# dataexplorations2026/cough_detector

Hardware: AMD Instinct MI355X
Metric: 1s@16kHz clips/sec (featurise+infer) (higher is better)
Workload: dtype bf16x3: split-bf16 MFMA (feature image, activations and BN-folded weights as hi+lo bf16 pairs, 3 v_mfma_f32_32x32x16_bf16 per k-step, f32 accumulate, f32 activations in HBM); featuriser f32

## Files before the change

### cough_detector_amd/csrc/resblock_x3.h

```cpp
#pragma once
#include <utility>

#include "common.h"
#include "nn_common.h"
#include "resnet_plan.h"

namespace cough {
namespace {

#ifdef COUGH_K1_STAMPS
__device__ unsigned long long* g_rb_stamp_buf = nullptr;
#define RB_STAMP(slot)                                                                        \
    do {                                                                                      \
        if (g_rb_stamp_buf && threadIdx.x == 0)                                               \
            g_rb_stamp_buf[(size_t)blockIdx.x * 8 + (slot)] = __builtin_amdgcn_s_memtime();   \
    } while (0)
#else
#define RB_STAMP(slot) do { } while (0)
#endif

struct RbxArgs {
    const float* x;
    int n_clips;
    const bf16_t* wf;
    const float* b1;
    const float* b2;
    float* out;
    const float* fcw;
    const float* fcb;
    float* logits;
    float* probs;
    int* preds;
    const int* nanflag;
};

template <int CIN, int COUT, int G, int XH, int XW>
struct RbxCfg {
    static constexpr int WAVES = 4, THREADS = 256;
    static constexpr bool T16 = rbx_t16(CIN, COUT, XH);
    static constexpr int OH = (XH - 1) / 2 + 1, OW = (XW - 1) / 2 + 1;
    static constexpr int NPX = XH * XW, PER = OH * OW, M = G * PER;
    static constexpr int NT = COUT / 32, MG = WAVES / NT, TILES = (M + 31) / 32;
    static constexpr int MW = (TILES + MG - 1) / MG;
    static constexpr int KS1 = 9 * CIN / 16, KSP = CIN / 16, KS2 = 9 * COUT / 16, KS = KS1 + KSP + KS2;
    static constexpr int CT = COUT / 16 / WAVES, NP = (M + 15) / 16;
    static constexpr int KQ1 = 9 * CIN / 32, KQP = CIN / 32, KQ2 = 9 * COUT / 32, KQ = KQ1 + KQP + KQ2;
    static_assert(!T16 || ((CT == 1 || CT == 2) && COUT == 16 * CT * WAVES && (CIN == 32 || CIN == 64) && G <= 2 &&
                           PER >= 16),
                  "T16: one or two 16-channel tiles per wave, one or two k32-steps per conv1 tap, at most one 16-pixel "
                  "tile straddling two clips");
    static constexpr int CHI = CIN / 8, CHO = COUT / 8;
    static constexpr int RE = (XH + 1) / 2, RO = XH / 2;
    static constexpr int NPP = 2 * XH * OW;
    static constexpr int PB01 = RE * OW, PB10 = 2 * RE * OW, PB11 = 2 * RE * OW + RO * OW;
    static constexpr int NPPC = T16 && G > 1 ? PER + (NPP - PER + 15) / 16 * 16 : NPP;
    static constexpr int ZC = T16 ? 16 : 1;
    static constexpr int CPX = !T16 ? (G * NPP + 1) * 16 : CHI == 4 ? (G * NPPC * 16 + 255) / 256 * 256 : (G * NPPC * 16 + 63) / 64 * 64;
    static constexpr int xoff(int c) {
        if (!T16 || CHI == 4) return c * CPX;
        const int s = (c & 1) * 4 + (c >> 1);
        return 256 + s * CPX + (s >= 2 ? 256 : 0) + (s >= 6 ? 256 : 0);
    }
    static constexpr int ZX = !T16 ? G * NPP * 16 : CHI == 4 ? 4 * CPX : 0;
    static constexpr int KX = T16 && CHI == 8 ? xoff(4) - xoff(0) : 0;
    static constexpr int ZH = T16 ? (M * 16 + 255) / 256 * 256 : M * 16;
    static constexpr int CPH = ZH + ZC * 16;
    static constexpr int XBYTES = !T16 ? CHI * CPX : CHI == 4 ? 4 * CPX + 256 : xoff(7) + CPX, HBYTES = CHO * CPH;
    static_assert(!T16 || (ZX % 256 == 0 && CPH % 256 == 0 && (G == 1 || (NPPC - PER) % 16 == 0)), "T16 bank residues");
    static_assert(!T16 || CHI == 4 || ((xoff(1) - xoff(0)) % 256 == 0 && (xoff(3) - xoff(2)) % 256 == 0 &&
                                       xoff(5) - xoff(1) == KX && xoff(6) - xoff(2) == KX && xoff(7) - xoff(3) == KX &&
                                       xoff(0) >= ZX + 256 && xoff(2) + CPX <= ZX + KX && xoff(4) >= ZX + KX + 256),
                  "T16 x layout, CIN = 64");
    static constexpr int PL = (((XBYTES > HBYTES ? XBYTES : HBYTES) + 255) / 256) * 256;
    static constexpr int BIAS = 2 * PL;
    static constexpr int HRED = BIAS + 2 * COUT * 4;
    static constexpr int LDS = HRED + WAVES * 2 * 4;
    static constexpr int OP = COUT + 4;
    static_assert(T16 || (WAVES % NT == 0 && MG * MW * 32 >= M), "tile split");
    static_assert(OW == (XW + 1) / 2, "sub-image row pitch");
    static_assert(M * OP * 4 <= 2 * PL, "the output tile lies over the planes");
    static constexpr int STAGE_MAX = 18;
    static_assert((G * NPX * CIN / 4 + THREADS - 1) / THREADS <= 2 * STAGE_MAX, "staging registers (f32 input, two batches)");
    static_assert(LDS <= 160 * 1024, "one workgroup must fit a CU");
    static_assert(LDS <= 80 * 1024 || (CIN == 32 && XH > 24) || (CIN == 64 && XH == 12), "two workgroups per CU");
};

template <int CIN, int COUT, int G, int XH, int XW>
__global__ __launch_bounds__(256, 2) void resblock_x3_kernel(RbxArgs a) {
    using Cfg = RbxCfg<CIN, COUT, G, XH, XW>;
    constexpr int THREADS = Cfg::THREADS, OH = Cfg::OH, OW = Cfg::OW, NPX = Cfg::NPX, PER = Cfg::PER, M = Cfg::M;
    constexpr bool T16 = Cfg::T16;
    using f32x4 = __attribute__((ext_vector_type(4))) float;
    constexpr int CHI = Cfg::CHI, CHO = Cfg::CHO, PL = Cfg::PL, OP = Cfg::OP, CPX = Cfg::CPX, CPH = Cfg::CPH, NPP = Cfg::NPP;
    constexpr int ZX = Cfg::ZX, KX = Cfg::KX, ZH = Cfg::ZH, ZC = Cfg::ZC, NPPC = Cfg::NPPC;
#ifndef RBX_D
#define RBX_D 4
#endif
#ifndef RBX_DQ
#define RBX_DQ 3
#endif
#ifndef RBX_P
#define RBX_P 2
#endif
#ifndef RBX_PRIO
#define RBX_PRIO 0
#endif
    extern __shared__ __attribute__((aligned(256))) char smem[];
    float* lbias = reinterpret_cast<float*>(smem + Cfg::BIAS);

    const int tid = threadIdx.x, lane = tid & 63, wave = tid >> 6;
    const int clip0 = blockIdx.x * G;
    const int nvalid = a.n_clips - clip0 < G ? a.n_clips - clip0 : G;
    RB_STAMP(0);

    float bv1 = 0.f, bv2 = 0.f;
    if (tid < COUT) { bv1 = a.b1[tid]; bv2 = a.b2[tid]; }

    constexpr int CT = T16 ? Cfg::CT : 1;
    constexpr int DW = !T16 ? RBX_D : CT == 2 && G == 1 ? 2 : RBX_DQ;
    const bf16_t* wbase = a.wf + size_t(T16 ? wave * CT : wave % Cfg::NT) * 1024 + lane * 8;
    constexpr int WSTEP = T16 ? COUT / 16 : Cfg::NT;
    auto wfrag = [&](int s, int ct, int plane) -> bf16x8 {
        return *reinterpret_cast<const bf16x8*>(wbase + ((size_t(s) * WSTEP + ct) * 2 + plane) * 512);
    };
    bf16x8 ring[DW][CT][2];
#pragma unroll
    for (int i = 0; i < DW; ++i)
#pragma unroll
        for (int ct = 0; ct < CT; ++ct) { ring[i][ct][0] = wfrag(i, ct, 0); ring[i][ct][1] = wfrag(i, ct, 1); }

    {
        constexpr int NPIECE = G * NPX * CIN / 4, UN = (NPIECE + THREADS - 1) / THREADS, QP = CIN / 4;
        constexpr int NB = UN <= Cfg::STAGE_MAX ? 1 : 2, UNB = (UN + NB - 1) / NB;
        const int valid = nvalid * NPX * QP;
        const float4* src = reinterpret_cast<const float4*>(a.x + (long long)clip0 * NPX * CIN);
        if constexpr (T16) {
            constexpr int NZ = CHI / 4;
            if (tid < 2 * NZ * ZC) {
                const int k = tid / ZC;
                *reinterpret_cast<uint4*>(smem + (k / NZ) * PL + ZX + (k % NZ) * KX + (tid % ZC) * 16) = make_uint4(0, 0, 0, 0);
            }
        } else if (tid < 2 * CHI) {
            *reinterpret_cast<uint4*>(smem + (tid / CHI) * PL + (tid % CHI) * CPX + ZX) = make_uint4(0, 0, 0, 0);
        }
#pragma unroll
        for (int b0 = 0; b0 < UN; b0 += UNB) {
            float4 v[UNB];
#pragma unroll
            for (int u = 0; u < UNB; ++u) {
                const int i = tid + (b0 + u) * THREADS;
                v[u] = src[i < valid ? i : valid - 1];
            }
#pragma unroll
            for (int u = 0; u < UNB; ++u) {
                const int i = tid + (b0 + u) * THREADS;
                if (i < NPIECE) {
                    const int P = i / QP, q = i % QP;
                    const int g = P / NPX, rem = P % NPX, ih = rem / XW, iw = rem % XW;
                    const int cell = g * NPPC + ((ih & 1) ? ((iw & 1) ? Cfg::PB11 : Cfg::PB10) : ((iw & 1) ? Cfg::PB01 : 0)) +
                                     (ih >> 1) * OW + (iw >> 1);
                    uint2 hi, lo;
                    if (i >= valid) v[u] = make_float4(0.f, 0.f, 0.f, 0.f);
                    split4(v[u].x, v[u].y, v[u].z, v[u].w, hi, lo);
                    const int off = Cfg::xoff(q >> 1) + cell * 16 + (q & 1) * 8;
                    *reinterpret_cast<uint2*>(smem + off) = hi;
                    *reinterpret_cast<uint2*>(smem + off + PL) = lo;
                }
            }
        }
    }
    if (tid < COUT) { lbias[tid] = bv1; lbias[COUT + tid] = bv2; }
    float fw0 = 0.f, fw1 = 0.f, fb0 = 0.f, fb1 = 0.f;
    if constexpr (COUT == 128) {
        if (a.fcw != nullptr) {
            fw0 = a.fcw[tid & 127]; fw1 = a.fcw[128 + (tid & 127)];
            fb0 = a.fcb[0]; fb1 = a.fcb[1];
        }
    }
    int nan_clip = 0;
    if constexpr (COUT == 128) {
        if (a.fcw != nullptr && a.nanflag != nullptr && (tid & 127) == 0 && (tid >> 7) < nvalid) nan_clip = a.nanflag[clip0 + (tid >> 7)];
    }

    auto tapx = [](int kh, int kw) constexpr -> int {
        const int a = (kh + 1) & 1, b = (kw + 1) & 1;
        return (a ? (b ? Cfg::PB11 : Cfg::PB10) : (b ? Cfg::PB01 : 0)) - (kh == 0 ? Cfg::OW : 0) - (kw == 0 ? 1 : 0);
    };

    constexpr int NT = Cfg::NT, MW = Cfg::MW, KS1 = Cfg::KS1, KSP = Cfg::KSP, KS = Cfg::KS, D = DW;
    const int r = lane & 31, h = lane >> 5, ng = wave % NT, mg = wave / NT;
    int goh[MW], gow[MW], px1[MW], ph1[MW];
    bool rok[MW];
#pragma unroll
    for (int mt = 0; mt < MW; ++mt) {
        const int R = (mg * MW + mt) * 32 + r;
        rok[mt] = R < M;
        const int Rc = rok[mt] ? R : 0;
        const int g = Rc / PER, rem = Rc % PER;
        goh[mt] = rok[mt] ? rem / OW : -4;
        gow[mt] = rem % OW;
        px1[mt] = (g * NPP + rem) * 16 + h * CPX;
        ph1[mt] = Rc * 16 + h * CPH;
    }

    constexpr int NP = Cfg::NP, KQ1 = Cfg::KQ1, KQP = Cfg::KQP, KQ = Cfg::KQ, P = RBX_P, NB = P + 1;
    constexpr int NI = KQ * NP, I2 = (KQ1 + KQP) * NP;
    const int px = lane & 15, tq = lane >> 4, n0 = 16 * CT * wave + 4 * tq;
    unsigned vm[NP];
#pragma unroll
    for (int t = 0; t < NP; ++t) {
        const int R = 16 * t + px, rem = G > 1 ? R % PER : R, oh = rem / OW, ow = rem % OW;
        unsigned m = 0;
#pragma unroll
        for (int tap = 0; tap < 9; ++tap) {
            const int kh = tap / 3, kw = tap % 3;
            const int ih = 2 * oh - 1 + kh, iw = 2 * ow - 1 + kw, jh = oh - 1 + kh, jw = ow - 1 + kw;
            if (unsigned(ih) < unsigned(XH) && unsigned(iw) < unsigned(XW)) m |= 1u << tap;
            if (unsigned(jh) < unsigned(OH) && unsigned(jw) < unsigned(OW)) m |= 1u << (9 + tap);
        }
        vm[t] = R < M ? m : 0u;
    }
    constexpr int DX = (NPPC - PER) * 16;
    const int lbx = px * 16 + Cfg::xoff(tq), lbh = px * 16 + tq * CPH, zh = ZH + tq * CPH;
    const int lbs = lbx + (G > 1 && px >= PER % 16 ? DX : 0);
    const int rx = px + (CHI == 4 ? 0 : Cfg::xoff(tq) / 16);
    auto zcell = [&](int z, int res) { return z + (res & 15) * 16; };
    RB_STAMP(1);
    __syncthreads();
    RB_STAMP(2);
#if RBX_PRIO
    __builtin_amdgcn_s_setprio(1);
#endif

    auto body16 = [&]() {
        f32x4 acc1[CT][NP], acc2[CT][NP];
#pragma unroll
        for (int ct = 0; ct < CT; ++ct)
#pragma unroll
            for (int t = 0; t < NP; ++t) { acc1[ct][t] = f32x4{0.f, 0.f, 0.f, 0.f}; acc2[ct][t] = f32x4{0.f, 0.f, 0.f, 0.f}; }

        int tadr[NP];
        auto aaddr = [&](auto ic) -> const char* {
            constexpr int i = decltype(ic)::value, q = i / NP, t = i % NP;
            constexpr bool conv1 = q < KQ1, proj = !conv1 && q < KQ1 + KQP;
            constexpr int kt = (conv1 ? q : proj ? q - KQ1 : q - KQ1 - KQP) * 32;
            constexpr int C = (conv1 || proj) ? CIN : COUT;
            constexpr int tap = proj ? 4 : kt / C, c32 = (kt % C) / 32, kh = tap / 3, kw = tap % 3;
            if constexpr (c32 == 0) {
                if constexpr (conv1 || proj) {
                    constexpr bool strad = G > 1 && 16 * t < PER && 16 * t + 16 > PER;
                    constexpr int off = 256 * t + (G > 1 && 16 * t >= PER ? DX : 0) + 16 * tapx(kh, kw);
                    tadr[t] = (vm[t] & (1u << tap)) ? (strad ? lbs : lbx) + off : zcell(ZX, rx + tapx(kh, kw));
                } else {
                    constexpr int off = 256 * t + 16 * ((kh - 1) * OW + kw - 1);
                    tadr[t] = (vm[t] & (1u << (9 + tap))) ? lbh + off : zcell(zh, px + (kh - 1) * OW + kw - 1);
                }
            }
            return smem + tadr[t] + c32 * ((conv1 || proj) ? KX : 4 * CPH);
        };
        bf16x8 af[NB][2];
        auto fetch = [&](auto ic) {
            constexpr int i = decltype(ic)::value;
            const char* p = aaddr(ic);
            af[i % NB][0] = *reinterpret_cast<const bf16x8*>(p);
            af[i % NB][1] = *reinterpret_cast<const bf16x8*>(p + PL);
        };
        [&]<int... Js>(std::integer_sequence<int, Js...>) {
            (fetch(std::integral_constant<int, Js>{}), ...);
        }(std::make_integer_sequence<int, P>{});

        auto pair = [&]<int i>() {
            constexpr int q = i / NP, t = i % NP, j = i + P;
            if constexpr (i == I2) {
                RB_STAMP(3);
#if RBX_PRIO
                __builtin_amdgcn_s_setprio(0);
#endif
                __syncthreads();
                for (int z = tid; z < 2 * CHO * ZC; z += THREADS) {
                    const int pl = z / ZC;
                    *reinterpret_cast<uint4*>(smem + (pl / CHO) * PL + (pl % CHO) * CPH + ZH + (z % ZC) * 16) =
                        make_uint4(0, 0, 0, 0);
                }
#pragma unroll
                for (int ct = 0; ct < CT; ++ct) {
                    const int n = n0 + 16 * ct;
                    const float4 bb = *reinterpret_cast<const float4*>(lbias + n);
#pragma unroll
                    for (int u = 0; u < NP; ++u) {
                        const int R = 16 * u + px;
                        uint2 hi, lo;
                        split4(fmaxf(acc1[ct][u][0] + bb.x, 0.f), fmaxf(acc1[ct][u][1] + bb.y, 0.f),
                               fmaxf(acc1[ct][u][2] + bb.z, 0.f), fmaxf(acc1[ct][u][3] + bb.w, 0.f), hi, lo);
                        if (R < M) {
                            const int off = (n >> 3) * CPH + R * 16 + ((n >> 2) & 1) * 8;
                            *reinterpret_cast<uint2*>(smem + off) = hi;
                            *reinterpret_cast<uint2*>(smem + off + PL) = lo;
                        }
                    }
                }
                __syncthreads();
                RB_STAMP(4);
#if RBX_PRIO
                __builtin_amdgcn_s_setprio(1);
#endif
                [&]<int... Js>(std::integer_sequence<int, Js...>) {
                    (fetch(std::integral_constant<int, I2 + Js>{}), ...);
                }(std::make_integer_sequence<int, P>{});
            }
            constexpr bool pf = j < NI && (j < I2) == (i < I2);
            constexpr bool wl = t == NP - 1 && q + DW < KQ;
            const bf16x8 cur_hi = af[i % NB][0], cur_lo = af[i % NB][1];
            const char* np = nullptr;
            if constexpr (pf) np = aaddr(std::integral_constant<int, j>{});
            [&]<int... Ms>(std::integer_sequence<int, Ms...>) {
                ([&] {
                    constexpr int m = Ms, kind = m / CT, ct = m % CT;
                    const bf16x8 w = ring[q % DW][ct][kind == 2 ? 1 : 0];
                    const bf16x8 x = kind == 1 ? cur_lo : cur_hi;
                    __builtin_amdgcn_sched_barrier(0);
                    if constexpr (q < KQ1) acc1[ct][t] = __builtin_amdgcn_mfma_f32_16x16x32_bf16(w, x, acc1[ct][t], 0, 0, 0);
                    else acc2[ct][t] = __builtin_amdgcn_mfma_f32_16x16x32_bf16(w, x, acc2[ct][t], 0, 0, 0);
                    __builtin_amdgcn_sched_barrier(0);
                    if constexpr (pf && m == CT - 1) af[j % NB][0] = *reinterpret_cast<const bf16x8*>(np);
                    if constexpr (pf && m == 2 * CT - 1) af[j % NB][1] = *reinterpret_cast<const bf16x8*>(np + PL);
                    if constexpr (wl && kind == 1) ring[q % DW][ct][0] = wfrag(q + DW, ct, 0);
                    if constexpr (wl && kind == 2) ring[q % DW][ct][1] = wfrag(q + DW, ct, 1);
                }(), ...);
            }(std::make_integer_sequence<int, 3 * CT>{});
            __builtin_amdgcn_sched_barrier(0);
        };
        [&]<int... Is>(std::integer_sequence<int, Is...>) {
            (pair.template operator()<Is>(), ...);
        }(std::make_integer_sequence<int, NI>{});

        RB_STAMP(5);
#if RBX_PRIO
        __builtin_amdgcn_s_setprio(0);
#endif
        __syncthreads();
        float* otile = reinterpret_cast<float*>(smem);
#pragma unroll
        for (int ct = 0; ct < CT; ++ct) {
            const int n = n0 + 16 * ct;
            const float4 bb = *reinterpret_cast<const float4*>(lbias + COUT + n);
#pragma unroll
            for (int t = 0; t < NP; ++t) {
                const int R = 16 * t + px;
                const float4 o = make_float4(fmaxf(acc2[ct][t][0] + bb.x, 0.f), fmaxf(acc2[ct][t][1] + bb.y, 0.f),
                                             fmaxf(acc2[ct][t][2] + bb.z, 0.f), fmaxf(acc2[ct][t][3] + bb.w, 0.f));
                if (R < M) *reinterpret_cast<float4*>(otile + R * OP + n) = o;
            }
        }
    };

    auto body = [&]<int MWX>() {
        f32x16 acc1[MWX], acc2[MWX];
#pragma unroll
        for (int mt = 0; mt < MWX; ++mt) { acc1[mt] = f32x16{0}; acc2[mt] = f32x16{0}; }

        int tadr[MWX];
        auto afrag = [&](auto sc, int mt, bf16x8& fhi, bf16x8& flo) {
            constexpr int s = decltype(sc)::value;
            constexpr bool conv1 = s < KS1, proj = !conv1 && s < KS1 + KSP;
            constexpr int kt = conv1 ? s * 16 : proj ? (s - KS1) * 16 : (s - KS1 - KSP) * 16;
            constexpr int C = (conv1 || proj) ? CIN : COUT, CP = (conv1 || proj) ? CPX : CPH;
            constexpr int tap = proj ? 4 : kt / C, c16 = (kt % C) / 16, kh = tap / 3, kw = tap % 3;
            if constexpr (c16 == 0) {
                if constexpr (conv1 || proj) {
                    const int ih = 2 * goh[mt] - 1 + kh, iw = 2 * gow[mt] - 1 + kw;
                    const bool ok = unsigned(ih) < unsigned(XH) && unsigned(iw) < unsigned(XW);
                    tadr[mt] = ok ? px1[mt] + tapx(kh, kw) * 16 : ZX + h * CPX;
                } else {
                    const int ih = goh[mt] - 1 + kh, iw = gow[mt] - 1 + kw;
                    const bool ok = unsigned(ih) < unsigned(OH) && unsigned(iw) < unsigned(OW);
                    tadr[mt] = ok ? ph1[mt] + ((kh - 1) * OW + kw - 1) * 16 : ZH + h * CPH;
                }
            }
            const char* p = smem + tadr[mt] + 2 * c16 * CP;
            fhi = *reinterpret_cast<const bf16x8*>(p);
            flo = *reinterpret_cast<const bf16x8*>(p + PL);
        };
        auto aaddr = [&](auto sc, int mt) -> const char* {
            constexpr int s = decltype(sc)::value;
            constexpr bool conv1 = s < KS1, proj = !conv1 && s < KS1 + KSP;
            constexpr int kt = conv1 ? s * 16 : proj ? (s - KS1) * 16 : (s - KS1 - KSP) * 16;
            constexpr int C = (conv1 || proj) ? CIN : COUT, CP = (conv1 || proj) ? CPX : CPH;
            constexpr int tap = proj ? 4 : kt / C, c16 = (kt % C) / 16, kh = tap / 3, kw = tap % 3;
            if constexpr (c16 == 0) {
                if constexpr (conv1 || proj) {
                    const int ih = 2 * goh[mt] - 1 + kh, iw = 2 * gow[mt] - 1 + kw;
                    const bool ok = unsigned(ih) < unsigned(XH) && unsigned(iw) < unsigned(XW);
                    tadr[mt] = ok ? px1[mt] + tapx(kh, kw) * 16 : ZX + h * CPX;
                } else {
                    const int ih = goh[mt] - 1 + kh, iw = gow[mt] - 1 + kw;
                    const bool ok = unsigned(ih) < unsigned(OH) && unsigned(iw) < unsigned(OW);
                    tadr[mt] = ok ? ph1[mt] + ((kh - 1) * OW + kw - 1) * 16 : ZH + h * CPH;
                }
            }
            return smem + tadr[mt] + 2 * c16 * CP;
        };

        bf16x8 af[2][MWX][2];
#pragma unroll
        for (int mt = 0; mt < MWX; ++mt) afrag(std::integral_constant<int, 0>{}, mt, af[0][mt][0], af[0][mt][1]);

        auto step = [&]<int s>() {
            if constexpr (s == KS1 + KSP) {
                RB_STAMP(3);
#if RBX_PRIO
                __builtin_amdgcn_s_setprio(0);
#endif
                __syncthreads();
                if (tid < 2 * CHO)
                    *reinterpret_cast<uint4*>(smem + (tid / CHO) * PL + (tid % CHO) * CPH + ZH) = make_uint4(0, 0, 0, 0);
#pragma unroll
                for (int mt = 0; mt < MWX; ++mt) {
                    const int R = (mg * MW + mt) * 32 + r;
#pragma unroll
                    for (int gq = 0; gq < 4; ++gq) {
                        const int n0 = ng * 32 + 8 * gq + 4 * h;
                        const float4 bb = *reinterpret_cast<const float4*>(lbias + n0);
                        uint2 hi, lo;
                        split4(fmaxf(acc1[mt][4 * gq] + bb.x, 0.f), fmaxf(acc1[mt][4 * gq + 1] + bb.y, 0.f),
                               fmaxf(acc1[mt][4 * gq + 2] + bb.z, 0.f), fmaxf(acc1[mt][4 * gq + 3] + bb.w, 0.f), hi, lo);
                        if (rok[mt]) {
                            const int off = (n0 >> 3) * CPH + R * 16 + h * 8;
                            *reinterpret_cast<uint2*>(smem + off) = hi;
                            *reinterpret_cast<uint2*>(smem + off + PL) = lo;
                        }
                    }
                }
                __syncthreads();
                RB_STAMP(4);
#if RBX_PRIO
                __builtin_amdgcn_s_setprio(1);
#endif
#pragma unroll
                for (int mt = 0; mt < MWX; ++mt)
                    afrag(std::integral_constant<int, s>{}, mt, af[s & 1][mt][0], af[s & 1][mt][1]);
            }
            const bf16x8 whi = ring[s % D][0][0], wlo = ring[s % D][0][1];
#pragma unroll
            for (int mt = 0; mt < MWX; ++mt) {
                constexpr bool pf = s + 1 < KS && s + 1 != KS1 + KSP;
                const bf16x8 cur_hi = af[s & 1][mt][0], cur_lo = af[s & 1][mt][1];
                const char* np = nullptr;
                if constexpr (pf) np = aaddr(std::integral_constant<int, s + 1>{}, mt);
                __builtin_amdgcn_sched_barrier(0);
                if constexpr (s < KS1) acc1[mt] = __builtin_amdgcn_mfma_f32_32x32x16_bf16(whi, cur_hi, acc1[mt], 0, 0, 0);
                else acc2[mt] = __builtin_amdgcn_mfma_f32_32x32x16_bf16(whi, cur_hi, acc2[mt], 0, 0, 0);
                __builtin_amdgcn_sched_barrier(0);
                if constexpr (pf) af[(s + 1) & 1][mt][0] = *reinterpret_cast<const bf16x8*>(np);
                if constexpr (s + D < KS) { if (mt == 0) ring[s % D][0][0] = wfrag(s + D, 0, 0); }
                __builtin_amdgcn_sched_barrier(0);
                if constexpr (s < KS1) acc1[mt] = __builtin_amdgcn_mfma_f32_32x32x16_bf16(whi, cur_lo, acc1[mt], 0, 0, 0);
                else acc2[mt] = __builtin_amdgcn_mfma_f32_32x32x16_bf16(whi, cur_lo, acc2[mt], 0, 0, 0);
                __builtin_amdgcn_sched_barrier(0);
                if constexpr (pf) af[(s + 1) & 1][mt][1] = *reinterpret_cast<const bf16x8*>(np + PL);
                if constexpr (s + D < KS) { if (mt == 0) ring[s % D][0][1] = wfrag(s + D, 0, 1); }
                __builtin_amdgcn_sched_barrier(0);
                if constexpr (s < KS1) acc1[mt] = __builtin_amdgcn_mfma_f32_32x32x16_bf16(wlo, cur_hi, acc1[mt], 0, 0, 0);
                else acc2[mt] = __builtin_amdgcn_mfma_f32_32x32x16_bf16(wlo, cur_hi, acc2[mt], 0, 0, 0);
                __builtin_amdgcn_sched_barrier(0);
            }
        };
        [&]<int... Ss>(std::integer_sequence<int, Ss...>) {
            (step.template operator()<Ss>(), ...);
        }(std::make_integer_sequence<int, KS>{});

        RB_STAMP(5);
#if RBX_PRIO
        __builtin_amdgcn_s_setprio(0);
#endif
        __syncthreads();
        float* otile = reinterpret_cast<float*>(smem);
#pragma unroll
        for (int mt = 0; mt < MWX; ++mt) {
            const int R = (mg * MW + mt) * 32 + r;
#pragma unroll
            for (int gq = 0; gq < 4; ++gq) {
                const int n0 = ng * 32 + 8 * gq + 4 * h;
                const float4 bb = *reinterpret_cast<const float4*>(lbias + COUT + n0);
                const float4 o = make_float4(fmaxf(acc2[mt][4 * gq] + bb.x, 0.f), fmaxf(acc2[mt][4 * gq + 1] + bb.y, 0.f),
                                             fmaxf(acc2[mt][4 * gq + 2] + bb.z, 0.f), fmaxf(acc2[mt][4 * gq + 3] + bb.w, 0.f));
                if (rok[mt]) *reinterpret_cast<float4*>(otile + R * OP + n0) = o;
            }
        }
    };
    constexpr int TILES = Cfg::TILES;
    const int mytiles = TILES - mg * MW < MW ? TILES - mg * MW : MW;
    if constexpr (T16) {
        body16();
    } else if constexpr (MW > 1 && TILES % MW != 0) {
        if (mytiles < MW) body.template operator()<(TILES % MW)>();
        else body.template operator()<MW>();
    } else {
        body.template operator()<MW>();
    }
    __syncthreads();
    RB_STAMP(6);
    const float* otile = reinterpret_cast<const float*>(smem);
    if (a.out != nullptr) {
        const int nvec = nvalid * PER * (COUT / 4);
        float4* o = reinterpret_cast<float4*>(a.out + (long long)clip0 * PER * COUT);
        for (int p = tid; p < nvec; p += THREADS) {
            const int row = p / (COUT / 4), c4 = p % (COUT / 4);
            o[p] = *reinterpret_cast<const float4*>(otile + row * OP + 4 * c4);
        }
    }
    if constexpr (COUT == 128) {
        static_assert(G * 128 <= THREADS, "one thread per (clip, channel)");
        if (a.fcw != nullptr) {
            float* hred = reinterpret_cast<float*>(smem + Cfg::HRED);
            const int c = tid & 127, g = tid >> 7;
            float sum = 0.f;
            if (g < G) {
#pragma unroll 6
                for (int i = 0; i < PER; ++i) sum += otile[(g * PER + i) * OP + c];
            }
            const float mean = sum / float(PER);
            float l0 = wave_sum(mean * fw0), l1 = wave_sum(mean * fw1);
            if (lane == 0) { hred[wave * 2] = l0; hred[wave * 2 + 1] = l1; }
            __syncthreads();
            if (c == 0 && g < nvalid) {
                const int w0 = g * 2;
                l0 = hred[w0 * 2] + hred[(w0 + 1) * 2] + fb0;
                l1 = hred[w0 * 2 + 1] + hred[(w0 + 1) * 2 + 1] + fb1;
                const long long b = clip0 + g;
                if (nan_clip) l0 = l1 = __builtin_nanf("");
                a.logits[b * 2] = l0;
                a.logits[b * 2 + 1] = l1;
                if (a.probs) {
                    const float mx = fmaxf(l0, l1), e0 = expf(l0 - mx), e1 = expf(l1 - mx), inv = 1.0f / (e0 + e1);
                    a.probs[b * 2] = e0 * inv;
                    a.probs[b * 2 + 1] = e1 * inv;
                }
                if (a.preds) a.preds[b] = (l1 > l0) ? 1 : 0;
            }
        }
    }
    RB_STAMP(7);
}

inline void pack_x3_fragments(std::vector<bf16_t>& wf, const std::vector<float>& w1, int K1, const std::vector<float>& wp,
                              int KP, const std::vector<float>& w2, int K2, int N) {
    const int nt = N / 32, ks1 = K1 / 16, ksp = KP / 16, ks2 = K2 / 16, ks = ks1 + ksp + ks2;
    wf.assign(size_t(ks) * nt * 2 * 512, 0);
    for (int s = 0; s < ks; ++s) {
        const std::vector<float>& w = s < ks1 ? w1 : s < ks1 + ksp ? wp : w2;
        const int K = s < ks1 ? K1 : s < ks1 + ksp ? KP : K2;
        const int sl = s < ks1 ? s : s < ks1 + ksp ? s - ks1 : s - ks1 - ksp;
        for (int t = 0; t < nt; ++t)
            for (int lane = 0; lane < 64; ++lane)
                for (int jj = 0; jj < 8; ++jj) {
                    const float v = w[size_t(32 * t + (lane & 31)) * K + 16 * sl + 8 * (lane >> 5) + jj];
                    const size_t base = ((size_t(s) * nt + t) * 2) * 512 + size_t(lane) * 8 + jj;
                    split_bf16_host(v, wf[base], wf[base + 512]);
                }
    }
}

inline void pack_x3_t16_fragments(std::vector<bf16_t>& wt, const std::vector<float>& w1, int K1, const std::vector<float>& wp,
                                   int KP, const std::vector<float>& w2, int K2, int N) {
    const int nt = N / 16, q1 = K1 / 32, qp = KP / 32, q2 = K2 / 32, nq = q1 + qp + q2;
    wt.assign(size_t(nq) * nt * 2 * 512, 0);
    for (int q = 0; q < nq; ++q) {
        const std::vector<float>& w = q < q1 ? w1 : q < q1 + qp ? wp : w2;
        const int K = q < q1 ? K1 : q < q1 + qp ? KP : K2;
        const int ql = q < q1 ? q : q < q1 + qp ? q - q1 : q - q1 - qp;
        for (int t = 0; t < nt; ++t)
            for (int lane = 0; lane < 64; ++lane)
                for (int jj = 0; jj < 8; ++jj) {
                    const float v = w[size_t(16 * t + (lane & 15)) * K + 32 * ql + 8 * (lane >> 4) + jj];
                    const size_t base = ((size_t(q) * nt + t) * 2) * 512 + size_t(lane) * 8 + jj;
                    split_bf16_host(v, wt[base], wt[base + 512]);
                }
    }
}

}
}
```

### cough_detector_amd/csrc/resnet_plan.h

```cpp
#pragma once
#include <cstddef>

namespace cough {
namespace {

constexpr int PLAN_FP32 = 0, PLAN_BF16 = 1, PLAN_BF16X3 = 3;

constexpr int NET_CH[3] = {32, 64, 128};

struct HW { int h, w; };
constexpr HW stem_out(HW i) { return {((i.h + 6 - 7) / 2 + 1) / 2, ((i.w + 6 - 7) / 2 + 1) / 2}; }
constexpr HW block_out(HW i) { return {(i.h + 2 - 3) / 2 + 1, (i.w + 2 - 3) / 2 + 1}; }

struct Shapes {
    int H, W;
    int P1h, P1w;
    int B0h, B0w;
    int B1h, B1w;
};
constexpr Shapes make_shapes(int H, int W) {
    const HW p1 = stem_out({H, W}), b0 = block_out(p1), b1 = block_out(b0);
    return {H, W, p1.h, p1.w, b0.h, b0.w, b1.h, b1.w};
}

constexpr size_t STEM_LDS_LIMIT = 64 * 1024;
constexpr int STEM_SB_MAXL = 22;
struct StemLds {
    int nrows, pitch;
    size_t bytes;
};
constexpr int plan_max(int a, int b) { return a > b ? a : b; }
constexpr StemLds stem_lds(const Shapes& s) {
    const int nrows = plan_max(4 * s.P1h + 6, s.H + 3), pitch = (plan_max(4 * s.P1w + 6, s.W + 3) + 1) & ~1;
    return {nrows, pitch, size_t(nrows) * pitch * 2};
}

constexpr int RBX_BLOCK0_ROWS[] = {16, 17, 22, 23, 24, 26, 27};
constexpr int RBX_BLOCK1_ROWS[] = {8, 9, 11, 12, 13, 14};
constexpr int RBX_COLS[2] = {25, 13};
constexpr int RBX_NROWS[2] = {int(sizeof(RBX_BLOCK0_ROWS) / sizeof(int)), int(sizeof(RBX_BLOCK1_ROWS) / sizeof(int))};
constexpr int rbx_rows(int blk, int i) { return blk == 0 ? RBX_BLOCK0_ROWS[i] : RBX_BLOCK1_ROWS[i]; }
constexpr int RBX_G_TALL = 1;
constexpr int rbx_block1_clips(int xh) { return xh <= 12 ? 2 : RBX_G_TALL; }
constexpr int rbx_clips(int blk, int xh) { return blk == 0 ? 1 : rbx_block1_clips(xh); }
constexpr int rbx_row(int blk, int xh, int xw) {
    if (xw != RBX_COLS[blk]) return -1;
    for (int i = 0; i < RBX_NROWS[blk]; ++i)
        if (rbx_rows(blk, i) == xh) return i;
    return -1;
}
constexpr bool rbx_compiled(int blk, int xh, int xw) { return rbx_row(blk, xh, xw) >= 0; }

constexpr bool rbx_t16_shape(int cin, int cout) { return (cin == 32 && cout == 64) || (cin == 64 && cout == 128); }
constexpr bool rbx_t16(int cin, int cout, int xh) {
    return rbx_t16_shape(cin, cout) && (cin == 64 || xh <= 26);
}

constexpr size_t RB_LDS_LIMIT = 160 * 1024;
struct RbParams { int cin, cout, g, mw, waves; };
constexpr RbParams RB_CFG[2] = {
    {32, 64, 1, 3, 4},
    {64, 128, 3, 2, 8}};
constexpr HW RB_FIXED[2] = {{22, 25}, {11, 13}};
static_assert(RB_CFG[0].cin == NET_CH[0] && RB_CFG[0].cout == NET_CH[1] && RB_CFG[1].cin == NET_CH[1] && RB_CFG[1].cout == NET_CH[2],
              "the block kernels' channels are the net's");
constexpr int rb_mtmax(RbParams p) { return p.waves / (p.cout / 32) * p.mw; }
constexpr int rb_threads(RbParams p) { return p.waves * 64; }
constexpr size_t rb_lds_bytes(RbParams p, int XH, int XW, int OH, int OW) {
    const size_t images = (size_t(p.g) * (XH + 2) * (XW + 2) * p.cin + size_t(p.g) * (OH + 2) * (OW + 2) * p.cout) * 2;
    const size_t tile = size_t(rb_mtmax(p)) * 32 * (p.cout + 8) * 2 + size_t(p.waves) * 2 * sizeof(float);
    return images > tile ? images : tile;
}
constexpr bool rb_fits(RbParams p, HW x, HW o) {
    return rb_lds_bytes(p, x.h, x.w, o.h, o.w) <= RB_LDS_LIMIT && p.g * o.h * o.w <= rb_mtmax(p) * 32 &&
           p.g * x.h * x.w * (p.cin / 8) <= 16 * rb_threads(p);
}

enum StemKernel { STEM_FEATURIZER , STEM_BF16, STEM_X3,
                  STEM_MFMA_F32, STEM_MFMA_BF16 };
enum BlockKernel { BLOCK_X3, BLOCK_BF16_FIXED, BLOCK_BF16_RUNTIME, BLOCK_CONV_MFMA, BLOCK_CONV_GEMM_BF16 };
enum BlockBody { BODY_32X32, BODY_16X16X32 };
enum HeadKernel { HEAD_FUSED , HEAD_TAIL_F32, HEAD_TAIL_BF16, HEAD_TAIL_GENERIC };
enum NanSource { NAN_FLAG , NAN_RESCAN  };

struct BlockPlan {
    BlockKernel kernel;
    BlockBody body;
    int clips;
    int nt;
    int row;
    size_t lds;
    HW in, out;
};
constexpr int PLAN_MAX_BLOCKS = 16;
struct NetPlan {
    bool ok;
    int n_blocks;
    StemKernel stem;
    StemLds stem_lds;
    HW stem_hw;
    BlockPlan block[PLAN_MAX_BLOCKS];
    HeadKernel head;
    NanSource nan;
    bool nan_in_block1;
    bool store_a3;
};

constexpr NetPlan plan_resnet(int dtype, bool shipped_channels, int n_blocks, int H, int W, bool stem_done) {
    NetPlan p{};
    p.n_blocks = n_blocks;
    p.stem_hw = stem_out({H, W});
    p.ok = p.stem_hw.h >= 1 && p.stem_hw.w >= 1;
    HW x = p.stem_hw;
    for (int i = 0; i < n_blocks; ++i) {
        BlockPlan& b = p.block[i];
        b.in = x;
        b.out = x = block_out(x);
        p.ok = p.ok && x.h >= 1 && x.w >= 1;
        b.kernel = BLOCK_CONV_MFMA;
        b.body = BODY_32X32;
        b.nt = 1;
        b.row = -1;
    }
    p.store_a3 = true;
    if (!shipped_channels) {
        p.stem = STEM_MFMA_F32;
        p.head = HEAD_TAIL_GENERIC;
        p.nan = NAN_RESCAN;
        return p;
    }
    const Shapes s = make_shapes(H, W);
    const StemLds l = stem_lds(s);
    const bool fits = H * W <= 2 * 256 * STEM_SB_MAXL;
    p.nan = NAN_FLAG;
    if (stem_done) {
        p.stem = STEM_FEATURIZER;
    } else if (dtype == PLAN_BF16 && l.bytes <= STEM_LDS_LIMIT && fits) {
        p.stem = STEM_BF16;
        p.stem_lds = l;
    } else if (dtype == PLAN_BF16X3 && 2 * l.bytes <= STEM_LDS_LIMIT && fits) {
        p.stem = STEM_X3;
        p.stem_lds = {l.nrows, l.pitch, 2 * l.bytes};
    } else {
        p.stem = dtype == PLAN_BF16 ? STEM_MFMA_BF16 : STEM_MFMA_F32;
        p.nan = NAN_RESCAN;
    }
    bool head_done = false;
    for (int i = 0; i < 2; ++i) {
        BlockPlan& b = p.block[i];
        const bool fused_x3 = dtype == PLAN_BF16X3 && rbx_compiled(i, b.in.h, b.in.w);
        const bool fused_bf16 = dtype == PLAN_BF16 && rb_fits(RB_CFG[i], b.in, b.out);
        if (fused_x3) {
            b.kernel = BLOCK_X3;
            b.body = rbx_t16(NET_CH[i], NET_CH[i + 1], b.in.h) ? BODY_16X16X32 : BODY_32X32;
            b.clips = rbx_clips(i, b.in.h);
            b.row = rbx_row(i, b.in.h, b.in.w);
            if (i == 1) p.nan_in_block1 = p.nan == NAN_FLAG;
        } else if (fused_bf16) {
            b.kernel = b.in.h == RB_FIXED[i].h && b.in.w == RB_FIXED[i].w ? BLOCK_BF16_FIXED : BLOCK_BF16_RUNTIME;
            b.clips = RB_CFG[i].g;
            b.lds = rb_lds_bytes(RB_CFG[i], b.in.h, b.in.w, b.out.h, b.out.w);
        } else {
            b.kernel = dtype == PLAN_BF16 ? BLOCK_CONV_GEMM_BF16 : BLOCK_CONV_MFMA;
            b.nt = NET_CH[i + 1] == 64 ? 2 : 4;
        }
        if (i == 1 && (fused_x3 || fused_bf16)) {
            head_done = true;
            p.store_a3 = !stem_done;
        }
    }
    p.head = head_done ? HEAD_FUSED : dtype == PLAN_BF16 ? HEAD_TAIL_BF16 : HEAD_TAIL_F32;
    return p;
}

constexpr const char* plan_name(StemKernel k) {
    switch (k) {
        case STEM_FEATURIZER: return "featurize_kernel";
        case STEM_BF16: return "stem_bf16<bf16>";
        case STEM_X3: return "stem_bf16<x3>";
        case STEM_MFMA_F32: return "stem_mfma<float>";
        case STEM_MFMA_BF16: return "stem_mfma<bf16>";
    }
    return "?";
}
constexpr const char* plan_name(const BlockPlan& b) {
    switch (b.kernel) {
        case BLOCK_X3: return "resblock_x3";
        case BLOCK_BF16_FIXED: return "resblock_bf16:fixed";
        case BLOCK_BF16_RUNTIME: return "resblock_bf16:runtime";
        case BLOCK_CONV_MFMA: return b.nt == 1 ? "conv_mfma<float,1>" : b.nt == 2 ? "conv_mfma<float,2>" : "conv_mfma<float,4>";
        case BLOCK_CONV_GEMM_BF16: return b.nt == 2 ? "conv_gemm_bf16<2>" : "conv_gemm_bf16<4>";
    }
    return "?";
}
constexpr const char* plan_name(BlockBody b) { return b == BODY_16X16X32 ? "16x16x32" : "32x32"; }
constexpr const char* plan_name(HeadKernel h) {
    switch (h) {
        case HEAD_FUSED: return "fused";
        case HEAD_TAIL_F32: return "tail_kernel<float>";
        case HEAD_TAIL_BF16: return "tail_kernel<bf16>";
        case HEAD_TAIL_GENERIC: return "tail_generic_kernel";
    }
    return "?";
}
constexpr const char* plan_name(NanSource n) { return n == NAN_FLAG ? "flag" : "rescan"; }

}
}
```

Measured before the change: 6.759 million.

## Use bordered zero-padded x planes in block-0 x3 resblock to drop conv1 tap masks

Adds a bordered layout for the parity-split input planes of the first fused x3 residual block. Explicit zero cells are written around each sub-image, so conv1 and projection taps always read valid (zero) data. The per-tap input bounds mask is then disabled and the A-operand address is computed directly from the tap offset. The border costs extra LDS and a zero-fill loop at kernel start. It is enabled only when the bordered layout still fits the same workgroups-per-CU LDS budget.

```diff
diff --git a/cough_detector_amd/csrc/resblock_x3.h b/cough_detector_amd/csrc/resblock_x3.h
--- a/cough_detector_amd/csrc/resblock_x3.h
+++ b/cough_detector_amd/csrc/resblock_x3.h
@@ -50,31 +50,35 @@
                   "T16: one or two 16-channel tiles per wave, one or two k32-steps per conv1 tap, at most one 16-pixel "
                   "tile straddling two clips");
     static constexpr int CHI = CIN / 8, CHO = COUT / 8;
-    static constexpr int RE = (XH + 1) / 2, RO = XH / 2;
-    static constexpr int NPP = 2 * XH * OW;
-    static constexpr int PB01 = RE * OW, PB10 = 2 * RE * OW, PB11 = 2 * RE * OW + RO * OW;
-    static constexpr int NPPC = T16 && G > 1 ? PER + (NPP - PER + 15) / 16 * 16 : NPP;
-    static constexpr int ZC = T16 ? 16 : 1;
-    static constexpr int CPX = !T16 ? (G * NPP + 1) * 16 : CHI == 4 ? (G * NPPC * 16 + 255) / 256 * 256 : (G * NPPC * 16 + 63) / 64 * 64;
-    static constexpr int xoff(int c) {
-        if (!T16 || CHI == 4) return c * CPX;
-        const int s = (c & 1) * 4 + (c >> 1);
-        return 256 + s * CPX + (s >= 2 ? 256 : 0) + (s >= 6 ? 256 : 0);
-    }
-    static constexpr int ZX = !T16 ? G * NPP * 16 : CHI == 4 ? 4 * CPX : 0;
-    static constexpr int KX = T16 && CHI == 8 ? xoff(4) - xoff(0) : 0;
-    static constexpr int ZH = T16 ? (M * 16 + 255) / 256 * 256 : M * 16;
-    static constexpr int CPH = ZH + ZC * 16;
-    static constexpr int XBYTES = !T16 ? CHI * CPX : CHI == 4 ? 4 * CPX + 256 : xoff(7) + CPX, HBYTES = CHO * CPH;
-    static_assert(!T16 || (ZX % 256 == 0 && CPH % 256 == 0 && (G == 1 || (NPPC - PER) % 16 == 0)), "T16 bank residues");
+    static constexpr RbxGeo L = rbx_geo(CIN, COUT, G, XH, XW);
+    static_assert(L.t16 == T16 && L.m == M && L.np == NP && L.chi == CHI && L.cho == CHO, "rbx_layout describes this instantiation");
+    static constexpr bool BX = L.border_x;
+    static constexpr int RE = L.re, RO = L.ro;
+    static constexpr int NPP = L.npp;
+    static constexpr int PB01 = L.b01, PB10 = L.b10, PB11 = L.b11;
+    static constexpr int NZX = BX ? rbx_x_nzero(RE, RO, OW) : 0;
+    static constexpr int NPPC = L.nppc;
+    static constexpr int ZC = L.zc;
+    static constexpr int CPX = L.cpx;
+    static constexpr int xoff(int c) { return rbx_xoff(T16, CHI, CPX, c); }
+    static constexpr int ZX = L.zx;
+    static constexpr int KX = L.kx;
+    static constexpr int ZH = L.zh;
+    static constexpr int CPH = L.cph;
+    static constexpr int XBYTES = L.xbytes, HBYTES = L.hbytes;
+    static_assert(!T16 || ((BX || ZX % 256 == 0) && CPX % (CHI == 4 ? 256 : 64) == 0 && CPH % 256 == 0 && (G == 1 || (NPPC - PER) % 16 == 0)),
+                  "T16 bank residues");
     static_assert(!T16 || CHI == 4 || ((xoff(1) - xoff(0)) % 256 == 0 && (xoff(3) - xoff(2)) % 256 == 0 &&
                                        xoff(5) - xoff(1) == KX && xoff(6) - xoff(2) == KX && xoff(7) - xoff(3) == KX &&
                                        xoff(0) >= ZX + 256 && xoff(2) + CPX <= ZX + KX && xoff(4) >= ZX + KX + 256),
                   "T16 x layout, CIN = 64");
-    static constexpr int PL = (((XBYTES > HBYTES ? XBYTES : HBYTES) + 255) / 256) * 256;
-    static constexpr int BIAS = 2 * PL;
-    static constexpr int HRED = BIAS + 2 * COUT * 4;
-    static constexpr int LDS = HRED + WAVES * 2 * 4;
+    static_assert(!BX || (T16 && CHI == 4 && G == 1 && XW % 2 == 1 && (16 * NP - 1 + PB11 + 1) * 16 <= CPX &&
+                          PB11 + RO * OW + (RE > RO ? OW : 0) <= NPP && PB01 % 8 >= 2 && (PB11 - PB10) % 8 >= 2),
+                  "bordered x planes");
+    static constexpr int PL = L.pl;
+    static constexpr int BIAS = L.bias;
+    static constexpr int HRED = L.hred;
+    static constexpr int LDS = L.lds;
     static constexpr int OP = COUT + 4;
     static_assert(T16 || (WAVES % NT == 0 && MG * MW * 32 >= M), "tile split");
     static_assert(OW == (XW + 1) / 2, "sub-image row pitch");
@@ -134,7 +138,14 @@
         constexpr int NB = UN <= Cfg::STAGE_MAX ? 1 : 2, UNB = (UN + NB - 1) / NB;
         const int valid = nvalid * NPX * QP;
         const float4* src = reinterpret_cast<const float4*>(a.x + (long long)clip0 * NPX * CIN);
-        if constexpr (T16) {
+        if constexpr (Cfg::BX) {
+            constexpr int NZX = Cfg::NZX;
+            for (int z = tid; z < 2 * CHI * NZX; z += THREADS) {
+                const int pl = z / NZX;
+                const int cell = rbx_x_zero(Cfg::PB01, Cfg::PB10, Cfg::PB11, OW, Cfg::RE, Cfg::RO, z % NZX);
+                *reinterpret_cast<uint4*>(smem + (pl / CHI) * PL + Cfg::xoff(pl % CHI) + cell * 16) = make_uint4(0, 0, 0, 0);
+            }
+        } else if constexpr (T16) {
             constexpr int NZ = CHI / 4;
             if (tid < 2 * NZ * ZC) {
                 const int k = tid / ZC;
@@ -157,8 +168,7 @@
                 if (i < NPIECE) {
                     const int P = i / QP, q = i % QP;
                     const int g = P / NPX, rem = P % NPX, ih = rem / XW, iw = rem % XW;
-                    const int cell = g * NPPC + ((ih & 1) ? ((iw & 1) ? Cfg::PB11 : Cfg::PB10) : ((iw & 1) ? Cfg::PB01 : 0)) +
-                                     (ih >> 1) * OW + (iw >> 1);
+                    const int cell = RBX_X_CELL(g * NPPC, Cfg::PB01, Cfg::PB10, Cfg::PB11, OW, ih, iw);
                     uint2 hi, lo;
                     if (i >= valid) v[u] = make_float4(0.f, 0.f, 0.f, 0.f);
                     split4(v[u].x, v[u].y, v[u].z, v[u].w, hi, lo);
@@ -182,10 +192,7 @@
         if (a.fcw != nullptr && a.nanflag != nullptr && (tid & 127) == 0 && (tid >> 7) < nvalid) nan_clip = a.nanflag[clip0 + (tid >> 7)];
     }
 
-    auto tapx = [](int kh, int kw) constexpr -> int {
-        const int a = (kh + 1) & 1, b = (kw + 1) & 1;
-        return (a ? (b ? Cfg::PB11 : Cfg::PB10) : (b ? Cfg::PB01 : 0)) - (kh == 0 ? Cfg::OW : 0) - (kw == 0 ? 1 : 0);
-    };
+    auto tapx = [](int kh, int kw) constexpr -> int { return rbx_x_tap(Cfg::PB01, Cfg::PB10, Cfg::PB11, Cfg::OW, kh, kw); };
 
     constexpr int NT = Cfg::NT, MW = Cfg::MW, KS1 = Cfg::KS1, KSP = Cfg::KSP, KS = Cfg::KS, D = DW;
     const int r = lane & 31, h = lane >> 5, ng = wave % NT, mg = wave / NT;
@@ -215,7 +222,7 @@
         for (int tap = 0; tap < 9; ++tap) {
             const int kh = tap / 3, kw = tap % 3;
             const int ih = 2 * oh - 1 + kh, iw = 2 * ow - 1 + kw, jh = oh - 1 + kh, jw = ow - 1 + kw;
-            if (unsigned(ih) < unsigned(XH) && unsigned(iw) < unsigned(XW)) m |= 1u << tap;
+            if (!Cfg::BX && unsigned(ih) < unsigned(XH) && unsigned(iw) < unsigned(XW)) m |= 1u << tap;
             if (unsigned(jh) < unsigned(OH) && unsigned(jw) < unsigned(OW)) m |= 1u << (9 + tap);
         }
         vm[t] = R < M ? m : 0u;
@@ -246,7 +253,9 @@
             constexpr int kt = (conv1 ? q : proj ? q - KQ1 : q - KQ1 - KQP) * 32;
             constexpr int C = (conv1 || proj) ? CIN : COUT;
             constexpr int tap = proj ? 4 : kt / C, c32 = (kt % C) / 32, kh = tap / 3, kw = tap % 3;
-            if constexpr (c32 == 0) {
+            if constexpr (Cfg::BX && (conv1 || proj)) {
+                return smem + lbx + (256 * t + 16 * tapx(kh, kw));
+            } else if constexpr (c32 == 0) {
                 if constexpr (conv1 || proj) {
                     constexpr bool strad = G > 1 && 16 * t < PER && 16 * t + 16 > PER;
                     constexpr int off = 256 * t + (G > 1 && 16 * t >= PER ? DX : 0) + 16 * tapx(kh, kw);
diff --git a/cough_detector_amd/csrc/resnet_plan.h b/cough_detector_amd/csrc/resnet_plan.h
--- a/cough_detector_amd/csrc/resnet_plan.h
+++ b/cough_detector_amd/csrc/resnet_plan.h
@@ -55,6 +55,99 @@
 constexpr bool rbx_t16(int cin, int cout, int xh) {
     return rbx_t16_shape(cin, cout) && (cin == 64 || xh <= 26);
 }
+
+constexpr int RBX_LDS_2WG = 80 * 1024, RBX_LDS_CU = 160 * 1024;
+constexpr int rbx_up(int v, int a) { return (v + a - 1) / a * a; }
+
+struct RbxGeo {
+    int cin, cout, g, xh, xw;
+    bool t16, border_x;
+    int oh, ow, npx, per, m, np;
+    int chi, cho, re, ro;
+    int b01, b10, b11;
+    int npp, nppc;
+    int zc, cpx, zx, kx;
+    int zh, cph;
+    int xbytes, hbytes, pl, bias, hred, lds;
+};
+
+constexpr int rbx_xoff(bool t16, int chi, int cpx, int c) {
+    if (!t16 || chi == 4) return c * cpx;
+    const int s = (c & 1) * 4 + (c >> 1);
+    return 256 + s * cpx + (s >= 2 ? 256 : 0) + (s >= 6 ? 256 : 0);
+}
+
+constexpr RbxGeo rbx_layout(int cin, int cout, int g, int xh, int xw, bool border_x) {
+    RbxGeo L{};
+    L.cin = cin; L.cout = cout; L.g = g; L.xh = xh; L.xw = xw;
+    L.t16 = rbx_t16(cin, cout, xh);
+    L.border_x = border_x;
+    L.oh = (xh - 1) / 2 + 1; L.ow = (xw - 1) / 2 + 1;
+    L.npx = xh * xw; L.per = L.oh * L.ow; L.m = g * L.per; L.np = (L.m + 15) / 16;
+    L.chi = cin / 8; L.cho = cout / 8; L.re = (xh + 1) / 2; L.ro = xh / 2;
+    L.zc = L.t16 ? 16 : 1;
+    if (border_x) {
+        L.b01 = L.re * L.ow + 1;
+        while (L.b01 % 8 < 2) ++L.b01;
+        L.b10 = L.b01 + L.re * L.ow + L.ow;
+        L.b11 = L.b10 + L.ro * L.ow + L.ow + 1;
+        L.npp = L.nppc = L.b11 + 16 * L.np;
+        L.cpx = rbx_up(L.npp * 16, 256);
+        L.zx = 0; L.kx = 0;
+        L.xbytes = L.chi * L.cpx;
+    } else {
+        L.b01 = L.re * L.ow; L.b10 = 2 * L.re * L.ow; L.b11 = 2 * L.re * L.ow + L.ro * L.ow;
+        L.npp = 2 * xh * L.ow;
+        L.nppc = L.t16 && g > 1 ? L.per + rbx_up(L.npp - L.per, 16) : L.npp;
+        L.cpx = !L.t16 ? (g * L.npp + 1) * 16 : L.chi == 4 ? rbx_up(g * L.nppc * 16, 256) : rbx_up(g * L.nppc * 16, 64);
+        L.zx = !L.t16 ? g * L.npp * 16 : L.chi == 4 ? 4 * L.cpx : 0;
+        L.kx = L.t16 && L.chi == 8 ? rbx_xoff(true, 8, L.cpx, 4) - rbx_xoff(true, 8, L.cpx, 0) : 0;
+        L.xbytes = !L.t16 ? L.chi * L.cpx : L.chi == 4 ? 4 * L.cpx + 256 : rbx_xoff(true, 8, L.cpx, 7) + L.cpx;
+    }
+    L.zh = L.t16 ? rbx_up(L.m * 16, 256) : L.m * 16;
+    L.cph = L.zh + L.zc * 16;
+    L.hbytes = L.cho * L.cph;
+    L.pl = rbx_up(L.xbytes > L.hbytes ? L.xbytes : L.hbytes, 256);
+    L.bias = 2 * L.pl;
+    L.hred = L.bias + 2 * cout * 4;
+    L.lds = L.hred + 4 * 2 * 4;
+    return L;
+}
+
+constexpr bool rbx_border_x(int blk, int xh) {
+    if (blk != 0 || !rbx_t16(NET_CH[0], NET_CH[1], xh) || RBX_COLS[0] % 2 == 0) return false;
+    const int sel = rbx_layout(NET_CH[0], NET_CH[1], 1, xh, RBX_COLS[0], false).lds;
+    const int bor = rbx_layout(NET_CH[0], NET_CH[1], 1, xh, RBX_COLS[0], true).lds;
+    return bor <= (sel <= RBX_LDS_2WG ? RBX_LDS_2WG : RBX_LDS_CU);
+}
+constexpr RbxGeo rbx_geo(int cin, int cout, int g, int xh, int xw) {
+    const bool bx = cin == NET_CH[0] && cout == NET_CH[1] && g == 1 && xw == RBX_COLS[0] && rbx_border_x(0, xh);
+    return rbx_layout(cin, cout, g, xh, xw, bx);
+}
+
+#define RBX_X_CELL(clip, b01, b10, b11, ow, ih, iw) \
+    ((clip) + (((ih) & 1) ? (((iw) & 1) ? (b11) : (b10)) : (((iw) & 1) ? (b01) : 0)) + ((ih) >> 1) * (ow) + ((iw) >> 1))
+constexpr int rbx_x_cell(int clip, int b01, int b10, int b11, int ow, int ih, int iw) { return RBX_X_CELL(clip, b01, b10, b11, ow, ih, iw); }
+constexpr int rbx_x_tap(int b01, int b10, int b11, int ow, int kh, int kw) {
+    const int a = (kh + 1) & 1, b = (kw + 1) & 1;
+    return (a ? (b ? b11 : b10) : (b ? b01 : 0)) - (kh == 0 ? ow : 0) - (kw == 0 ? 1 : 0);
+}
+constexpr int rbx_x_nzero(int re, int ro, int ow) { return re + ro + 1 + ow + ow + 1 + (re > ro ? ow : 0); }
+constexpr int rbx_x_zero(int b01, int b10, int b11, int ow, int re, int ro, int k) {
+    if (k < re) return b01 + k * ow + ow - 1;
+    k -= re;
+    if (k < ro) return b11 + k * ow + ow - 1;
+    k -= ro;
+    if (k < 1) return b01 - 1;
+    k -= 1;
+    if (k < ow) return b10 - ow + k;
+    k -= ow;
+    if (k < ow + 1) return b10 + ro * ow + k;
+    k -= ow + 1;
+    return b11 + ro * ow + k;
+}
+constexpr int rbx_h_cell(int R) { return R; }
+constexpr int rbx_h_tap(int ow, int kh, int kw) { return (kh - 1) * ow + kw - 1; }
 
 constexpr size_t RB_LDS_LIMIT = 160 * 1024;
 struct RbParams { int cin, cout, g, mw, waves; };
```

Result: faster. 6.890 million, median of 6 (+1.9%).
